# EspressoSystems/Push-CDN

Measured on AMD Instinct MI355X. Metric: broadcast_msgs_per_sec, higher is better.
Workload: dtype uint8; 1 GPU; model=gpu-broker-mesh, payload_bytes=1024, subscribers_total=10000, subscribers_per_broker=10000, topics=8, mode=broadcast, population=all, drops=0, parallelism=single-broker, global_batch=256, seq_len=1024

## Files before the change

### csrc/gpu_bindings.cpp

```cpp

#include <torch/extension.h>
#include <ATen/hip/HIPContext.h>
#include <hip/hip_runtime.h>

#include <cstdint>

#include "hip/bls_kernels.h"
#include "hip/dataplane.h"

#define CHECK_DEV(x) TORCH_CHECK(x.is_cuda(), #x " must be on the GPU")
#define CHECK_CONTIG(x) TORCH_CHECK(x.is_contiguous(), #x " must be contiguous")

static inline PairRec* pair_ptr(torch::Tensor& pairs) {
    TORCH_CHECK(pairs.dim() == 2 && pairs.size(1) == 4 && pairs.dtype() == torch::kInt32
                && pairs.is_contiguous(), "pairs must be a contiguous int32 [cap, 4] tensor");
    return (PairRec*)pairs.data_ptr<int32_t>();
}

static inline hipStream_t cur_stream() {
    return at::hip::getCurrentHIPStream().stream();
}

static inline torch::TensorOptions opts(torch::ScalarType dtype, const torch::Tensor& like) {
    return torch::TensorOptions().dtype(dtype).device(like.device());
// ... 374 lines not shown
    TORCH_CHECK(n_users >= 0 && n_peers >= 0 && ring_wpos.numel() >= n_users + n_peers,
                "ring_wpos must cover n_users + n_peers rings");
    int32_t capacity = (int32_t)pairs.size(0);
    launch_k5b_emit_direct_peers(
        disc.data_ptr<int32_t>(), owner.data_ptr<int32_t>(), origin.data_ptr<int32_t>(),
        payload_off.data_ptr<int64_t>(), payload_len.data_ptr<int32_t>(), M,
        (int32_t)n_users, (int32_t)n_peers, ring_bytes, capacity,
        (uint64_t*)ring_wpos.data_ptr<int64_t>(), n_pairs.data_ptr<int32_t>(),
        pair_ptr(pairs), (uint32_t*)drops.data_ptr<int32_t>(), cur_stream());
}

void direct_apply(torch::Tensor table_keys, torch::Tensor table_vals, torch::Tensor up_keys,
                  torch::Tensor up_owners, torch::Tensor del_keys, torch::Tensor n_failed) {
    CHECK_DEV(table_keys); CHECK_DEV(table_vals); CHECK_DEV(up_keys); CHECK_DEV(up_owners);
    CHECK_DEV(del_keys); CHECK_DEV(n_failed);
    CHECK_CONTIG(table_keys); CHECK_CONTIG(table_vals); CHECK_CONTIG(up_keys);
    CHECK_CONTIG(up_owners); CHECK_CONTIG(del_keys);
    int64_t S = table_keys.size(0);
    TORCH_CHECK(S > 0 && (S & (S - 1)) == 0, "table size must be a power of two");
    TORCH_CHECK(table_vals.numel() == S && table_keys.dtype() == torch::kInt64
                && table_vals.dtype() == torch::kInt32);
    TORCH_CHECK(up_keys.dtype() == torch::kInt64 && del_keys.dtype() == torch::kInt64
                && up_owners.dtype() == torch::kInt32 && n_failed.dtype() == torch::kInt32);
    TORCH_CHECK(up_owners.numel() == up_keys.numel() && n_failed.numel() >= 1);
    launch_k6_direct_apply((uint64_t*)table_keys.data_ptr<int64_t>(),
                           table_vals.data_ptr<int32_t>(), S,
                           (const uint64_t*)up_keys.data_ptr<int64_t>(),
                           up_owners.data_ptr<int32_t>(), (int32_t)up_keys.numel(),
                           (const uint64_t*)del_keys.data_ptr<int64_t>(),
                           (int32_t)del_keys.numel(),
                           (uint32_t*)n_failed.data_ptr<int32_t>(), cur_stream());
}

PYBIND11_MODULE(TORCH_EXTENSION_NAME, m) {
    m.def("topic_mask_origin_t", &topic_mask_origin_t,
          "K2a transposed with per-message origin: remote-origin rows keep user bits only");
    m.def("emit_direct_peers", &emit_direct_peers,
          "K5b with peer recipient slots (owner -(p+2) -> ring n_users+p, local origin only)");
    m.def("direct_apply", &direct_apply,
          "K6: batched DirectMap upserts/deletes on the device table");
    m.def("parse_batch", &parse_batch, "K4: on-device capnp parse of a message batch",
          py::arg("buf"), py::arg("offsets"), py::arg("hash_seed") = 0);
    m.def("topic_mask", &topic_mask, "K2a: per-message subscriber mask");
    m.def("assign_emit", &assign_emit, "K2b: per-user FIFO ring assignment + pair list");
    m.def("fanout", &fanout, "K3: N-way payload fan-out into egress rings");
    m.def("direct_lookup", &direct_lookup, "K5: batched direct-route hash probe");
    m.def("apply_subs", &apply_subs, "K2c: apply subscribe/unsubscribe batch to bitmap");
    m.def("bls_verify_batch", &bls_verify_batch, "K1: batched BLS-over-BN254 verification");
    m.def("compact_rings", &compact_rings,
          "K7: gather used egress-ring prefixes into one staging buffer");
    m.def("precompute_g2_lines", &precompute_g2_lines,
          "fixed-g2 Miller line coefficients for K1 v2 (once per process)");
    m.def("bls_verify_batch2", &bls_verify_batch2,
          "K1 v2: 2-lane Fp2-decomposed batched BLS verification");
    m.def("_k1_dbg_wave",
          [](torch::Tensor vks, torch::Tensor sigs, torch::Tensor msgs, torch::Tensor moff,
             torch::Tensor g2_lines, torch::Tensor rand_r, int64_t mode) {
              int32_t N = (int32_t)moff.size(0) - 1;
              auto ok = torch::zeros({N}, opts(torch::kInt32, vks));
              launch_k1_dbg_wave(vks.data_ptr<uint8_t>(), sigs.data_ptr<uint8_t>(),
                                 msgs.data_ptr<uint8_t>(), moff.data_ptr<int64_t>(),
                                 g2_lines.data_ptr<uint8_t>(),
                                 (const uint64_t*)rand_r.data_ptr<int64_t>(), N,
                                 (int32_t)mode, ok.data_ptr<int32_t>(), cur_stream());
              return ok;
          });
    m.def("bls_verify_batch_wave", &bls_verify_batch_wave,
// ... 18 lines not shown
```

### csrc/hip/dataplane.h

```cpp
#pragma once

#include <hip/hip_runtime_api.h>
#include <stdint.h>

struct alignas(16) PairRec { int32_t user; int32_t msg; int64_t dst; };
static_assert(sizeof(PairRec) == 16, "PairRec must be one dword4");

struct ParseOut {
    int32_t* disc;
    int64_t* payload_off;
    int32_t* payload_len;
    int64_t* topics_off;
    int32_t* topics_cnt;
    uint64_t* recip_hash;
    uint64_t* timestamp;
};

extern "C" {

void launch_k4_parse(const uint8_t* buf, const int64_t* offsets, int32_t M, uint64_t hash_seed,
                     ParseOut out, hipStream_t s);

void launch_k2a_topic_mask(const uint64_t* sub_bitmap, const uint8_t* buf,
                           const int64_t* topics_off, const int32_t* topics_cnt,
                           const int32_t* disc, uint64_t* mask, int32_t M, int32_t W,
                           hipStream_t s);
void launch_k2a_topic_mask_t(const uint64_t* sub_bitmap, const uint8_t* buf,
                             const int64_t* topics_off, const int32_t* topics_cnt,
                             const int32_t* disc, uint64_t* mask_t, int32_t M, int32_t W,
                             hipStream_t s);
void launch_k2a_topic_mask_origin_t(const uint64_t* sub_bitmap, const uint8_t* buf,
                                    const int64_t* topics_off, const int32_t* topics_cnt,
                                    const int32_t* disc, const int32_t* origin,
                                    uint64_t* mask_t, int32_t M, int32_t W, int32_t n_users,
                                    hipStream_t s);
void launch_k2c_apply_subs(uint64_t* sub_bitmap, const uint8_t* buf, const int64_t* topics_off,
                           const int32_t* topics_cnt, const int32_t* disc,
                           const int32_t* user_idx, int32_t M, int32_t W, hipStream_t s);

void launch_k2b_count(const uint64_t* mask, int32_t M, int32_t W, int32_t n_users,
                      int32_t* counts, hipStream_t s);
void launch_k2b_emit(const uint64_t* mask, const int64_t* payload_off,
                     const int32_t* payload_len, const int32_t* pair_base, int32_t M, int32_t W,
                     int32_t n_users, int64_t ring_bytes, uint64_t* ring_wpos, PairRec* pairs,
                     uint32_t* drops, hipStream_t s);
void launch_k2b_fused_t(const uint64_t* mask_t, const int32_t* payload_len, int32_t M,
                        int32_t W, int32_t n_users, int64_t ring_bytes, int32_t capacity,
                        int32_t uniform_rec, uint64_t* ring_wpos, int32_t* n_pairs,
// ... 16 lines not shown
                          const uint32_t* msg_seq, const int32_t* n_pairs_ptr,
                          int32_t capacity, int32_t ref_threshold, int64_t ref_base,
                          uint8_t* egress, int nt, int grid, hipStream_t s);
void launch_k3_fanout_flat2(const uint8_t* buf, const int64_t* payload_off,
                            const int32_t* payload_len, const PairRec* pairs,
                            uint32_t seq_base, const int32_t* n_pairs_ptr, int32_t capacity,
                            int32_t units_per_pair, int32_t uniform_len, uint8_t* egress,
                            int nt, int grid, hipStream_t s);
void launch_k3_fanout_flat3(const uint8_t* buf, const int64_t* payload_off,
                            const int32_t* payload_len, const PairRec* pairs,
                            const uint32_t* seq_state, const int32_t* n_pairs_ptr,
                            int32_t capacity, int32_t units_per_pair, int32_t uniform_len,
                            uint8_t* egress, int nt, int grid, hipStream_t s);
void launch_k_seq_advance(uint32_t* seq_state, int32_t m, hipStream_t s);

void launch_k5_direct_lookup(const uint64_t* table_keys, const int32_t* table_vals,
                             int64_t table_size, const uint64_t* query, int32_t N,
                             int32_t* owner, hipStream_t s);
void launch_k5b_emit_direct(const int32_t* disc, const int32_t* owner,
                            const int64_t* payload_off, const int32_t* payload_len, int32_t M,
                            int64_t ring_bytes, int32_t capacity, uint64_t* ring_wpos,
                            int32_t* n_pairs, PairRec* pairs, uint32_t* drops, hipStream_t s);
void launch_k5b_emit_direct_peers(const int32_t* disc, const int32_t* owner,
                                  const int32_t* origin, const int64_t* payload_off,
                                  const int32_t* payload_len, int32_t M, int32_t n_users,
                                  int32_t n_peers, int64_t ring_bytes, int32_t capacity,
                                  uint64_t* ring_wpos, int32_t* n_pairs, PairRec* pairs,
                                  uint32_t* drops, hipStream_t s);
void launch_k6_direct_apply(uint64_t* table_keys, int32_t* table_vals, int64_t table_size,
                            const uint64_t* up_keys, const int32_t* up_owners, int32_t n_up,
                            const uint64_t* del_keys, int32_t n_del, uint32_t* n_failed,
                            hipStream_t s);

void launch_k7_compact_rings(const uint8_t* egress, int64_t ring_bytes, const int64_t* wpos,
                             const int64_t* dst_off, uint8_t* staging, int32_t n_rings,
                             int32_t max_chunks, hipStream_t s);

}
```

### csrc/hip/dataplane.hip

```cpp

#include <hip/hip_runtime.h>
#include <stdint.h>

#include "../common/divmagic.h"
#include "dataplane.h"

#define WAVE 64
#ifndef CDN_CHECK
#define CDN_CHECK 1
#endif

#define RING_ALIGN 16ull
__host__ __device__ inline uint64_t ring_rec(int32_t len) {
    return ((uint64_t)len + 16 + (RING_ALIGN - 1)) & ~(RING_ALIGN - 1);
}

typedef unsigned int cdn_v4u __attribute__((ext_vector_type(4)));
template <int NT>
__device__ __forceinline__ void store16(void* dst, cdn_v4u v) {
    if (NT) __builtin_nontemporal_store(v, (cdn_v4u*)dst);
    else *(cdn_v4u*)dst = v;
}

__device__ __forceinline__ void store_pair(PairRec* p, int32_t u, int32_t m, int64_t d) {
// ... 502 lines not shown
            store16<NT>(egress + dsto, cdn_v4u{(uint32_t)len | REF_FLAG, seq, (uint32_t)ro,
                                               (uint32_t)(ro >> 32)});
        }
        unsigned long long inl = __ballot(live && !by_ref);
        while (inl) {
            const int j = __ffsll((long long)inl) - 1;
            inl &= inl - 1;
            const int32_t jlen = __shfl(len, j);
            const uint32_t jseq = (uint32_t)__shfl((int)seq, j);
            const int64_t joff = ((int64_t)__shfl((int)(off >> 32), j) << 32)
                                 | (uint32_t)__shfl((int)off, j);
            const int64_t jdst = ((int64_t)__shfl((int)(dsto >> 32), j) << 32)
                                 | (uint32_t)__shfl((int)dsto, j);
            copy_record<NT>(egress + jdst, buf + joff, jlen, jseq, lane, WAVE);
        }
    }
}

extern "C" {

void launch_k3_fanout_ref(const uint8_t* buf, const int64_t* payload_off,
                          const int32_t* payload_len, const PairRec* pairs,
                          const uint32_t* msg_seq, const int32_t* n_pairs_ptr,
                          int32_t capacity, int32_t ref_threshold, int64_t ref_base,
                          uint8_t* egress, int nt, int grid, hipStream_t s) {
    if (grid <= 0) grid = 4096;
    DISPATCH_NT(nt, hipLaunchKernelGGL((k3_fanout_ref_t<NT>), dim3(grid), dim3(256), 0, s, buf,
                                       payload_off, payload_len, pairs, msg_seq, n_pairs_ptr,
                                       capacity, ref_threshold, ref_base, egress));
}

}

template <int NT, bool SEQ_FROM_PTR>
__global__ void __launch_bounds__(256) k3_fanout_flat_t(
    const uint8_t* __restrict__ buf,
    const int64_t* __restrict__ payload_off,
    const int32_t* __restrict__ payload_len,
    const PairRec* __restrict__ pairs,
    uint32_t seq_base_val,
    const uint32_t* __restrict__ seq_state,
    const int32_t* __restrict__ n_pairs_ptr,
    int32_t capacity,
    int32_t units_per_pair,
    uint32_t div_magic,
    int32_t div_shift,
    int32_t uniform_len,
    uint8_t* __restrict__ egress)
{
    const uint32_t seq_base = SEQ_FROM_PTR ? seq_state[0] : seq_base_val;
    int np = *n_pairs_ptr;
    if (np > capacity) np = capacity;
    const int64_t n_units = (int64_t)np * units_per_pair;
    const int64_t stride = (int64_t)gridDim.x * blockDim.x;
    for (int64_t f = (int64_t)blockIdx.x * blockDim.x + threadIdx.x; f < n_units; f += stride) {
        const uint32_t f32 = (uint32_t)f;
        const int p = (int)(((uint64_t)f32 * div_magic) >> div_shift);
        const int unit = (int)(f32 - (uint32_t)p * (uint32_t)units_per_pair);
        const PairRec pr = pairs[p];
        if (pr.user < 0) continue;
        const int mi = pr.msg;
        const int32_t len = uniform_len > 0 ? uniform_len : payload_len[mi];
        uint8_t* dst = egress + pr.dst + (size_t)unit * 16;
        if (unit == 0) {
            store16<NT>(dst, cdn_v4u{(uint32_t)len, seq_base + (uint32_t)mi, 0u, 0u});
            continue;
        }
        const uint8_t* src = buf + payload_off[mi] + (size_t)(unit - 1) * 16;
        const int32_t coff = (unit - 1) * 16;
        if (coff + 16 <= len && (((uintptr_t)src) & 15) == 0) {
            store16<NT>(dst, *(const cdn_v4u*)src);
        } else if (coff >= len) {
            store16<NT>(dst, cdn_v4u{0u, 0u, 0u, 0u});
        } else {
            uint8_t tmp[16];
            #pragma unroll
            for (int b = 0; b < 16; ++b) tmp[b] = (coff + b < len) ? src[b] : 0;
            cdn_v4u v; memcpy(&v, tmp, 16);
            store16<NT>(dst, v);
        }
    }
}


template <bool SEQ_FROM_PTR>
static void launch_flat(const uint8_t* buf, const int64_t* payload_off,
                        const int32_t* payload_len, const PairRec* pairs, uint32_t seq_base,
                        const uint32_t* seq_state, const int32_t* n_pairs_ptr, int32_t capacity,
                        int32_t units_per_pair, int32_t uniform_len, uint8_t* egress, int nt,
                        int grid, hipStream_t s) {
    if (grid <= 0) grid = 16384;
    uint32_t dm; int32_t dsh;
    u32_div_magic(units_per_pair, &dm, &dsh);
    DISPATCH_NT(nt, hipLaunchKernelGGL((k3_fanout_flat_t<NT, SEQ_FROM_PTR>), dim3(grid),
                                       dim3(256), 0, s, buf, payload_off, payload_len, pairs,
                                       seq_base, seq_state, n_pairs_ptr, capacity,
                                       units_per_pair, dm, dsh, uniform_len, egress));
}

extern "C" __global__ void k_seq_advance(uint32_t* seq_state, int32_t m) {
    if (blockIdx.x == 0 && threadIdx.x == 0) seq_state[0] += (uint32_t)m;
}

extern "C" {

void launch_k3_fanout_flat2(const uint8_t* buf, const int64_t* payload_off,
                            const int32_t* payload_len, const PairRec* pairs,
                            uint32_t seq_base, const int32_t* n_pairs_ptr, int32_t capacity,
                            int32_t units_per_pair, int32_t uniform_len, uint8_t* egress,
                            int nt, int grid, hipStream_t s) {
    launch_flat<false>(buf, payload_off, payload_len, pairs, seq_base, nullptr, n_pairs_ptr,
                       capacity, units_per_pair, uniform_len, egress, nt, grid, s);
}
// ... 92 lines not shown

    uint64_t wpos = ring_wpos[u];
    uint32_t dropped = 0;
    for (int m = 0; m < M; ++m) {
        if (!(col[m] & bit)) continue;
        int32_t len = payload_len[m];
        uint64_t rec = ring_rec(len);
        bool fits_ring = (wpos + rec <= (uint64_t)ring_bytes);
        bool fits_cap = (slot < capacity);
        if (!fits_ring || !fits_cap) {
            if (fits_cap) { store_pair(pairs + slot, -1, m, 0); slot++; }
            dropped++;
            continue;
        }
        store_pair(pairs + slot, u, m, (int64_t)u * ring_bytes + wpos);
        slot++;
        wpos += rec;
    }
    ring_wpos[u] = wpos;
    if (dropped) atomicAdd(drops, dropped);
}

extern "C" {

void launch_k2a_topic_mask_t(const uint64_t* sub_bitmap, const uint8_t* buf,
                             const int64_t* topics_off, const int32_t* topics_cnt,
                             const int32_t* disc, uint64_t* mask_t, int32_t M, int32_t W,
                             hipStream_t s) {
    if (M <= 0) return;
    hipLaunchKernelGGL(k2a_topic_mask_t, k2a_grid(M, W), dim3(K2A_THREADS), 0, s, sub_bitmap,
                       buf, topics_off, topics_cnt, disc, mask_t, M, W);
}

#define K2B_BLK 32

extern "C" __global__ void k2b_p1_count(
    const uint64_t* __restrict__ mask_t,
    int32_t M, int32_t W, int32_t NB,
    int32_t* __restrict__ bcount)
{
    const int wave = (blockIdx.x * blockDim.x + threadIdx.x) >> 6;
    if (wave >= W * NB) return;
    const int w = wave / NB, b = wave - (int64_t)(wave / NB) * NB;
    const int lane = threadIdx.x & 63;
    const uint64_t bit = 1ull << lane;
    const uint64_t* col = mask_t + (int64_t)w * M;
    const int m0 = b * K2B_BLK, m1 = min(M, m0 + K2B_BLK);
    int c = 0;
    for (int m = m0; m < m1; ++m) c += (col[m] & bit) ? 1 : 0;
    bcount[(int64_t)b * (W * 64) + (w * 64 + lane)] = c;
}

extern "C" __global__ void k2b_p2_bases(
    const int32_t* __restrict__ bcount,
    int32_t W, int32_t NB, int32_t n_users,
    int64_t ring_bytes, int32_t capacity, int32_t uniform_rec,
    uint64_t* __restrict__ ring_wpos,
    int32_t* __restrict__ n_pairs,
    int32_t* __restrict__ pprefix,
    int32_t* __restrict__ ubase,
    int32_t* __restrict__ ufit,
    int64_t* __restrict__ udst,
    uint32_t* __restrict__ drops)
{
    const int u = blockIdx.x * blockDim.x + threadIdx.x;
    const bool active = u < n_users;
    const int lane = threadIdx.x & 63;
    int total = 0;
    if (active) {
        for (int b = 0; b < NB; ++b) {
            pprefix[(int64_t)b * (W * 64) + u] = total;
            total += bcount[(int64_t)b * (W * 64) + u];
        }
    }
    const int my_base = wave_claim_span(total, n_pairs);
    uint32_t dropped = 0;
    if (active) {
        ubase[u] = my_base;
        const uint64_t wpos = ring_wpos[u];
        const int32_t fit = (int32_t)((ring_bytes - wpos) / (uint64_t)uniform_rec);
        ufit[u] = fit;
        udst[u] = (int64_t)u * ring_bytes + (int64_t)wpos;
        int cap_room = capacity - my_base; if (cap_room < 0) cap_room = 0;
        int emitted = total; if (emitted > fit) emitted = fit; if (emitted > cap_room) emitted = cap_room;
        ring_wpos[u] = wpos + (uint64_t)emitted * uniform_rec;
        dropped = (uint32_t)(total - emitted);
    }
    for (int d = 1; d < 64; d <<= 1) dropped += __shfl_down(dropped, d);
    if (lane == 0 && dropped) atomicAdd(drops, dropped);
}

extern "C" __global__ void k2b_p3_emit(
    const uint64_t* __restrict__ mask_t,
    const int32_t* __restrict__ pprefix,
    const int32_t* __restrict__ ubase,
    const int32_t* __restrict__ ufit,
    const int64_t* __restrict__ udst,
    int32_t M, int32_t W, int32_t NB, int32_t n_users,
    int32_t capacity, int32_t uniform_rec,
    PairRec* __restrict__ pairs)
{
    const int wave = (blockIdx.x * blockDim.x + threadIdx.x) >> 6;
    if (wave >= W * NB) return;
    const int w = wave / NB, b = wave - (int64_t)(wave / NB) * NB;
    const int lane = threadIdx.x & 63;
    const int u = w * 64 + lane;
    if (u >= n_users) return;
    const uint64_t bit = 1ull << lane;
    const uint64_t* col = mask_t + (int64_t)w * M;
    int p = pprefix[(int64_t)b * (W * 64) + u];
    const int base = ubase[u], fit = ufit[u];
    const int64_t dstb = udst[u];
    const int m0 = b * K2B_BLK, m1 = min(M, m0 + K2B_BLK);
    for (int m = m0; m < m1; ++m) {
        if (!(col[m] & bit)) continue;
        const int slot = base + p;
        if (slot < capacity) {
            if (p < fit)
                store_pair(pairs + slot, u, m, dstb + (int64_t)p * uniform_rec);
            else
                store_pair(pairs + slot, -1, m, 0);
        }
// ... 228 lines not shown
                                    uint64_t* mask_t, int32_t M, int32_t W, int32_t n_users,
                                    hipStream_t s) {
    if (M <= 0) return;
    hipLaunchKernelGGL(k2a_topic_mask_origin_t, k2a_grid(M, W), dim3(K2A_THREADS), 0, s,
                       sub_bitmap, buf, topics_off, topics_cnt, disc, origin, mask_t, M, W,
                       n_users);
}

void launch_k5b_emit_direct_peers(
    const int32_t* disc, const int32_t* owner, const int32_t* origin,
    const int64_t* payload_off, const int32_t* payload_len, int32_t M, int32_t n_users,
    int32_t n_peers, int64_t ring_bytes, int32_t capacity, uint64_t* ring_wpos,
    int32_t* n_pairs, PairRec* pairs, uint32_t* drops, hipStream_t s) {
    if (M <= 0) return;
    int threads = 256, blocks = (M + threads - 1) / threads;
    hipLaunchKernelGGL(k5b_emit_direct_peers, dim3(blocks), dim3(threads), 0, s, disc, owner,
                       origin, payload_off, payload_len, M, n_users, n_peers, ring_bytes,
                       capacity, ring_wpos, n_pairs, pairs, drops);
}

void launch_k6_direct_apply(uint64_t* table_keys, int32_t* table_vals, int64_t table_size,
                            const uint64_t* up_keys, const int32_t* up_owners, int32_t n_up,
                            const uint64_t* del_keys, int32_t n_del, uint32_t* n_failed,
                            hipStream_t s) {
    const int total = n_up + n_del;
    if (total <= 0) return;
    int threads = 256, blocks = (total + threads - 1) / threads;
    hipLaunchKernelGGL(k6_direct_apply, dim3(blocks), dim3(threads), 0, s, table_keys,
                       table_vals, table_size, up_keys, up_owners, n_up, del_keys, n_del,
                       n_failed);
}

}
```

### pushcdn_amd/broker/gpu_engine.py

```python

from __future__ import annotations

import os

from dataclasses import dataclass
from typing import Dict, List, Optional, Tuple

import torch

from ..utils.keyhash import fnv1a64
from ..utils.log import get_logger

log = get_logger("gpu-engine")

RING_ALIGN = 16
REF_FLAG = 0x80000000


def ring_rec(length: int) -> int:
    return (length + 16 + (RING_ALIGN - 1)) & ~(RING_ALIGN - 1)


@dataclass
class TickStats:
    n_messages: int = 0
    n_broadcast: int = 0
    n_direct: int = 0
    n_deliveries: int = 0
    n_drops: int = 0


class GpuBrokerEngine:
    def __init__(
        self,
        device: str = "cuda:0",
        n_users: int = 10_000,
        ring_bytes: int = 1 << 21,
        direct_table_size: int = 1 << 16,
        use_gpu_ops: Optional[bool] = None,
        fanout_wire: bool = False,
        pair_capacity: int = 4 << 20,
        nt_fanout: bool = True,
        direct_enabled: bool = True,
        hash_seed: int = 0,
        n_peer_slots: int = 0,
        ref_threshold: Optional[int] = None,
    ) -> None:
        assert n_peer_slots >= 0
        self.n_peer_slots = n_peer_slots
        self.n_recipients = n_users + n_peer_slots
        self.pair_capacity = pair_capacity
        self._flat_max_rec = int(os.environ.get("PUSHCDN_FLAT_MAX_REC", "4096"))
        flat_units = self._flat_max_rec // 16 + 1
        assert 1 <= flat_units <= (1 << 21), "PUSHCDN_FLAT_MAX_REC too large"
        assert pair_capacity * flat_units < (1 << 31), (
            f"pair_capacity {pair_capacity} x {flat_units} flat units/record "
            "must stay below 2^31")
        self.nt_fanout = nt_fanout
        self.direct_enabled = direct_enabled
        self.hash_seed = hash_seed & ((1 << 64) - 1)
        self.fanout_wire = fanout_wire
        self.device = torch.device(device)
        self.is_cuda = self.device.type == "cuda"
        if use_gpu_ops is None:
            use_gpu_ops = self.is_cuda
        self.use_gpu_ops = use_gpu_ops
        if self.use_gpu_ops:
            from ..ops import get_gpu_ops

            self._ops = get_gpu_ops()
        else:
            self._ops = None

        assert ring_bytes % 16 == 0
        self.n_users = n_users
        self.ring_bytes = ring_bytes
        R = self.n_recipients
        self.W = (R + 63) // 64

        dev = self.device
        self.sub_bitmap = torch.zeros((256, self.W), dtype=torch.int64, device=dev)
        self.egress = torch.zeros(R * ring_bytes, dtype=torch.uint8, device=dev)
        self.ring_wpos = torch.zeros(R, dtype=torch.int64, device=dev)
        self.direct_keys = torch.zeros(direct_table_size, dtype=torch.int64, device=dev)
        self.direct_vals = torch.zeros(direct_table_size, dtype=torch.int32, device=dev)
        self._direct_entries: Dict[int, int] = {}
        self._direct_pubkeys: Dict[int, bytes] = {}
        self._direct_tombstones: set = set()
        self._direct_failed = torch.zeros(1, dtype=torch.int32, device=dev)
        if ref_threshold is not None:
            assert fanout_wire, "ref_threshold requires fanout_wire=True"
            assert 1 <= ref_threshold < REF_FLAG
            assert ring_rec(ref_threshold - 1) <= ring_bytes, (
                f"ref_threshold {ref_threshold}: an inline message just below it "
                f"does not fit a {ring_bytes}-byte ring")
        self.ref_threshold = ref_threshold
        self._ref_batches: List[bytes] = []
        self._ref_base = 0
        self.seq = 0
        self.total = TickStats()
        self._staging_dev: Optional[torch.Tensor] = None
        self._staging_host: Optional[torch.Tensor] = None
        if self.use_gpu_ops:
            o32 = dict(dtype=torch.int32, device=dev)
            self._pairs = torch.empty((pair_capacity, 4), **o32)
            self._drops = torch.zeros(1, **o32)
            self._n_pairs = torch.zeros(1, **o32)
            self._seq_dev = torch.zeros(1, **o32)
            self._graphs: Dict[Tuple[int, int, int], object] = {}


    def subscribe(self, user_idx: int, topics: List[int]) -> None:
        w, bit = user_idx >> 6, 1 << (user_idx & 63)
        bit = bit - (1 << 64) if bit >= (1 << 63) else bit
        for t in topics:
            self.sub_bitmap[t & 0xFF, w] |= bit

    def unsubscribe(self, user_idx: int, topics: List[int]) -> None:
        w, bit = user_idx >> 6, 1 << (user_idx & 63)
        bit = bit - (1 << 64) if bit >= (1 << 63) else bit
        for t in topics:
            self.sub_bitmap[t & 0xFF, w] &= ~bit

    def subscribe_all(self, topics: List[int]) -> None:
        if self.n_peer_slots:
            full = self._user_bit_words().to(self.device)
            for t in topics:
                self.sub_bitmap[t & 0xFF] |= full
            return
        full = torch.full((self.W,), -1, dtype=torch.int64)
        tail = self.n_users & 63
        if tail:
            full[-1] = (1 << tail) - 1
        for t in topics:
            self.sub_bitmap[t & 0xFF] = full.to(self.device)

    def _user_bit_words(self) -> torch.Tensor:
        words = torch.zeros(self.W, dtype=torch.int64)
        nfull = self.n_users >> 6
        words[:nfull] = -1
        tail = self.n_users & 63
# ... 201 lines not shown
        self._ref_base = 0

    def _k2b_block_scratch(self, M: int):
        NB = (M + 31) // 32
        W64 = self.W * 64
        cur = getattr(self, "_k2b_scratch", None)
        if cur is not None and cur[0] >= NB:
            return cur[1]
        o32 = dict(dtype=torch.int32, device=self.device)
        bufs = (
            torch.empty(NB * W64, **o32),
            torch.empty(NB * W64, **o32),
            torch.empty(W64, **o32),
            torch.empty(W64, **o32),
            torch.empty(W64, dtype=torch.int64, device=self.device),
        )
        self._k2b_scratch = (NB, bufs)
        return bufs

    def _assign_emit(self, ops, mask_t, payload_len, rec: int, M: int) -> None:
        if rec and self.use_gpu_ops:
            bcount, pprefix, ubase, ufit, udst = self._k2b_block_scratch(M)
            ops.assign_emit_blocks_t(
                mask_t, self.ring_wpos, self.ring_bytes, self.n_recipients,
                bcount, pprefix, ubase, ufit, udst,
                self._pairs, self._drops, self._n_pairs, rec,
            )
        else:
            ops.assign_emit_fused_t(
                mask_t, payload_len, self.ring_wpos, self.ring_bytes, self.n_recipients,
                self._pairs, self._drops, self._n_pairs, rec,
            )

    def _tick_gpu(self, buf: torch.Tensor, offsets: torch.Tensor,
                  uniform_wire_len: Optional[int] = None, origin=None,
                  ref_base: int = 0) -> TickStats:
        ops = self._ops
        M = offsets.shape[0] - 1
        disc, payload_off, payload_len, topics_off, topics_cnt, recip_hash, _ts = ops.parse_batch(
            buf, offsets, self.hash_seed
        )
        peer_plane = self.n_peer_slots > 0 or origin is not None
        if peer_plane:
            origin = self._origin_tensor(origin, M)
            mask_t = ops.topic_mask_origin_t(self.sub_bitmap, buf, topics_off, topics_cnt,
                                             disc, origin, self.n_users)
        else:
            mask_t = ops.topic_mask_t(self.sub_bitmap, buf, topics_off, topics_cnt, disc)
        if self.fanout_wire:
            payload_off = offsets[:-1].contiguous()
            payload_len = (offsets[1:] - offsets[:-1]).to(torch.int32).contiguous()
        self._n_pairs.zero_()
        uniform = self.fanout_wire and uniform_wire_len is not None
        thr = self.ref_threshold
        ring_len = payload_len
        if thr is not None:
            if uniform and uniform_wire_len >= thr:
                uniform = False
            if not uniform:
                ring_len = torch.where(payload_len >= thr, 0, payload_len).to(torch.int32)
        rec = ring_rec(uniform_wire_len) if uniform else 0
        self._assign_emit(ops, mask_t, ring_len, rec, M)
        if self.direct_enabled:
            owner = ops.direct_lookup(self.direct_keys, self.direct_vals, recip_hash)
            if peer_plane:
                ops.emit_direct_peers(disc, owner, origin, payload_off, ring_len,
                                      self.ring_bytes, self.n_users, self.n_peer_slots,
                                      self.ring_wpos, self._n_pairs, self._pairs,
                                      self._drops)
            else:
                ops.emit_direct(disc, owner, payload_off, ring_len, self.ring_bytes,
# ... 76 lines not shown
                torch.tensor(offsets[1:], dtype=torch.int64)
                - torch.tensor(offsets[:-1], dtype=torch.int64)
            ).to(torch.int32)
        thr = self.ref_threshold
        ring_len = pr.payload_len if thr is None else ref.ring_lengths(pr.payload_len, thr)

        def fan(p_user, p_msg, p_dst):
            if thr is None:
                ref.fanout(batch, pr.payload_off, pr.payload_len, p_user, p_msg, p_dst,
                           seq, arr)
            else:
                ref.fanout_ref(batch, pr.payload_off, pr.payload_len, p_user, p_msg, p_dst,
                               seq, arr, thr, ref_base)

        pair_user, pair_msg, pair_dst, drops = ref.assign_emit(
            mask, ring_len, self.ring_wpos, self.ring_bytes, self.n_recipients
        )
        seq = torch.arange(self.seq, self.seq + M, dtype=torch.int32)
        self.seq += M
        arr = bytearray(self.egress.numpy().tobytes())
        fan(pair_user, pair_msg, pair_dst)
        owner = ref.direct_lookup(self.direct_keys, self.direct_vals, pr.recip_hash)
        d_user, d_msg, d_dst, d_drops = ref.emit_direct_peers(
            pr.disc, owner, origin, ring_len, self.ring_wpos, self.ring_bytes,
            self.n_users, self.n_peer_slots)
        fan(d_user, d_msg, d_dst)
        self.egress.copy_(torch.frombuffer(arr, dtype=torch.uint8))
        return TickStats(n_messages=M, n_deliveries=int(pair_user.shape[0]),
                         n_drops=drops + d_drops)


    def drain_cursors(self) -> torch.Tensor:
        self._discard_ref_batches()
        wpos = self.ring_wpos.detach().clone().to("cpu")
        self.ring_wpos.zero_()
        return wpos

    def drain_compact(self) -> Tuple[torch.Tensor, torch.Tensor, torch.Tensor]:
        self._discard_ref_batches()
        return self._drain_compact()

    def drain_compact_ref(self):
        batches = self._ref_batches
        self._discard_ref_batches()
        if len(batches) == 1:
            refbuf = batches[0]
        else:
            refbuf = b"".join(bytes(b) for b in batches)
        return (*self._drain_compact(), refbuf)

    def _drain_compact(self) -> Tuple[torch.Tensor, torch.Tensor, torch.Tensor]:
        if not self.use_gpu_ops:
            wpos = self.ring_wpos.detach().clone()
            self.ring_wpos.zero_()
            offsets = torch.zeros(self.n_recipients + 1, dtype=torch.int64)
            torch.cumsum(wpos, 0, out=offsets[1:])
            total = int(offsets[-1])
            staging = torch.empty(total, dtype=torch.uint8)
            for u in range(self.n_recipients):
                n = int(wpos[u])
                if n:
                    s = u * self.ring_bytes
                    staging[int(offsets[u]):int(offsets[u + 1])] = self.egress[s:s + n]
            return wpos, offsets, staging
        wpos_dev = self.ring_wpos
        wpos = wpos_dev.detach().to("cpu")
# ... 65 lines not shown
```

Before: 393,600 msgs/s.

## Add fused uniform broadcast tick with dense tile fan-out and fused cursor drain

Adds a single host entry point that runs parse, topic mask, per-tile k2b assignment and fan-out back to back from preallocated scratch, so the per-tick Python dispatch and tensor allocation go away. Fully subscribed 32-message tiles are written as a dense image broadcast to every user's ring, and only leftover tiles are emitted as sparse pairs. Cursor drain becomes one kernel plus a pinned async copy. Tick stats no longer report deliveries or drops, and the path applies only to uniform, non-direct, non-peer ticks.

```diff
diff --git a/csrc/common/tick_geom.h b/csrc/common/tick_geom.h
--- /dev/null
+++ b/csrc/common/tick_geom.h
@@ -0,0 +1,29 @@
+#pragma once
+
+#include <stdint.h>
+
+#define K2B_BLK 32
+
+#define DENSE_THREADS 256
+#define DENSE_MAX_V 8
+#define DENSE_GROUP 8
+struct DenseGeom { int32_t n_chunks; int32_t chunk_units; };
+static inline DenseGeom dense_geom(int32_t units_per_rec) {
+    const int32_t cap = DENSE_THREADS * DENSE_MAX_V;
+    const int32_t image = units_per_rec * K2B_BLK;
+    DenseGeom g;
+    g.n_chunks = (image + cap - 1) / cap;
+    g.chunk_units = ((image + g.n_chunks - 1) / g.n_chunks + 63) & ~63;
+    return g;
+}
+static inline int64_t dense_grid_x(int32_t n_users, int32_t group, int32_t n_chunks) {
+    return ((int64_t)n_users + group - 1) / group * n_chunks;
+}
+
+static inline int64_t k2b_blocks(int64_t M) { return (M + K2B_BLK - 1) / K2B_BLK; }
+static inline int64_t uniform_tick_scratch64(int64_t M, int64_t W, int64_t units_per_rec) {
+    return 4 * M + W * M + k2b_blocks(M) * W * 64 + W * 64 + 2 * M * units_per_rec;
+}
+static inline int64_t uniform_tick_scratch32(int64_t M, int64_t W) {
+    return 3 * M + 3 * k2b_blocks(M) * W * 64 + 2 * W * 64;
+}
diff --git a/csrc/gpu_bindings.cpp b/csrc/gpu_bindings.cpp
--- a/csrc/gpu_bindings.cpp
+++ b/csrc/gpu_bindings.cpp
@@ -430,7 +430,97 @@
                            (uint32_t*)n_failed.data_ptr<int32_t>(), cur_stream());
 }
 
+void tick_uniform_broadcast(torch::Tensor buf, torch::Tensor offsets, uint64_t hash_seed,
+                            torch::Tensor sub_bitmap, torch::Tensor ring_wpos,
+                            int64_t ring_bytes, int64_t n_users, torch::Tensor pairs,
+                            torch::Tensor drops, torch::Tensor n_pairs, torch::Tensor n_sparse,
+                            torch::Tensor scratch64, torch::Tensor scratch32,
+                            int64_t uniform_len, int64_t seq_base, torch::Tensor egress,
+                            int64_t nt, int64_t dense) {
+    CHECK_DEV(buf); CHECK_CONTIG(buf); CHECK_DEV(offsets); CHECK_CONTIG(offsets);
+    CHECK_DEV(sub_bitmap); CHECK_CONTIG(sub_bitmap); CHECK_DEV(ring_wpos); CHECK_CONTIG(ring_wpos);
+    CHECK_DEV(egress); CHECK_CONTIG(egress); CHECK_DEV(scratch64); CHECK_DEV(scratch32);
+    CHECK_DEV(drops); CHECK_DEV(n_pairs); CHECK_DEV(n_sparse);
+    TORCH_CHECK(buf.dtype() == torch::kUInt8 && offsets.dtype() == torch::kInt64
+                && egress.dtype() == torch::kUInt8);
+    TORCH_CHECK(sub_bitmap.dim() == 2 && sub_bitmap.size(0) == 256);
+    const int64_t M = offsets.size(0) - 1, W = sub_bitmap.size(1);
+    if (M <= 0) return;
+    TORCH_CHECK(uniform_len >= 0 && uniform_len < (int64_t(1) << 30));
+    const int64_t rec = (uniform_len + 16 + 15) & ~int64_t(15);
+    TORCH_CHECK(ring_bytes % 16 == 0 && n_users >= 0 && n_users <= W * 64
+                && ring_wpos.numel() >= n_users && ring_wpos.dtype() == torch::kInt64
+                && egress.numel() >= n_users * ring_bytes,
+                "rings do not cover n_users");
+    TORCH_CHECK(buf.numel() >= M * uniform_len, "batch shorter than M uniform messages");
+    check_flat_shape(pairs, rec / 16);
+    TORCH_CHECK(M * (rec / 16) < (int64_t(1) << 31)
+                && dense_grid_x((int32_t)n_users, DENSE_GROUP, dense_geom((int32_t)(rec / 16)).n_chunks)
+                       * k2b_blocks(M) < (int64_t(1) << 31),
+                "batch too large for the dense fan-out");
+    TORCH_CHECK(scratch64.dtype() == torch::kInt64 && scratch32.dtype() == torch::kInt32
+                && scratch64.is_contiguous() && scratch32.is_contiguous()
+                && (uintptr_t)scratch64.data_ptr<int64_t>() % 16 == 0
+                && scratch64.numel() >= uniform_tick_scratch64(M, W, rec / 16)
+                && scratch32.numel() >= uniform_tick_scratch32(M, W),
+                "fused tick scratch too small");
+    UniformTick t;
+    t.buf = buf.data_ptr<uint8_t>();
+    t.offsets = offsets.data_ptr<int64_t>();
+    t.M = (int32_t)M;
+    t.hash_seed = hash_seed;
+    t.sub_bitmap = (const uint64_t*)sub_bitmap.data_ptr<int64_t>();
+    t.W = (int32_t)W;
+    t.n_users = (int32_t)n_users;
+    t.ring_bytes = ring_bytes;
+    t.capacity = (int32_t)pairs.size(0);
+    t.uniform_len = (int32_t)uniform_len;
+    t.rec = (int32_t)rec;
+    t.seq_base = (uint32_t)seq_base;
+    t.ring_wpos = (uint64_t*)ring_wpos.data_ptr<int64_t>();
+    t.n_pairs = n_pairs.data_ptr<int32_t>();
+    t.n_sparse = n_sparse.data_ptr<int32_t>();
+    t.pairs = pair_ptr(pairs);
+    t.drops = (uint32_t*)drops.data_ptr<int32_t>();
+    t.scratch64 = scratch64.data_ptr<int64_t>();
+    t.scratch32 = scratch32.data_ptr<int32_t>();
+    t.egress = egress.data_ptr<uint8_t>();
+    t.nt = (int)nt;
+    t.dense = (int)dense;
+    launch_tick_uniform_broadcast(&t, cur_stream());
+}
+
+std::vector<int64_t> uniform_tick_scratch_sizes(int64_t M, int64_t W, int64_t rec) {
+    return {uniform_tick_scratch64(M, W, rec / 16), uniform_tick_scratch32(M, W)};
+}
+
+void drain_cursors(torch::Tensor ring_wpos, torch::Tensor staging, torch::Tensor host) {
+    CHECK_DEV(ring_wpos); CHECK_CONTIG(ring_wpos); CHECK_DEV(staging); CHECK_CONTIG(staging);
+    TORCH_CHECK(!host.is_cuda() && host.is_pinned() && host.is_contiguous(),
+                "host must be a pinned CPU tensor");
+    TORCH_CHECK(ring_wpos.dtype() == torch::kInt64 && staging.dtype() == torch::kInt64
+                && host.dtype() == torch::kInt64);
+    const int64_t n = ring_wpos.numel();
+    TORCH_CHECK(staging.numel() >= n && host.numel() >= n && n <= INT32_MAX);
+    if (n == 0) return;
+    hipStream_t s = cur_stream();
+    launch_drain_cursors(ring_wpos.data_ptr<int64_t>(), staging.data_ptr<int64_t>(), (int32_t)n,
+                         s);
+    hipError_t e = hipMemcpyAsync(host.data_ptr<int64_t>(), staging.data_ptr<int64_t>(),
+                                  (size_t)n * 8, hipMemcpyDeviceToHost, s);
+    TORCH_CHECK(e == hipSuccess, "drain_cursors copy: ", hipGetErrorString(e));
+    e = hipStreamSynchronize(s);
+    TORCH_CHECK(e == hipSuccess, "drain_cursors sync: ", hipGetErrorString(e));
+}
+
 PYBIND11_MODULE(TORCH_EXTENSION_NAME, m) {
+    m.def("tick_uniform_broadcast", &tick_uniform_broadcast,
+          "fused uniform broadcast tick: K4, K2a, K2b tiles, dense + sparse fan-out");
+    m.def("uniform_tick_scratch_sizes", &uniform_tick_scratch_sizes,
+          "(int64, int32) scratch elements tick_uniform_broadcast needs for (M, W, rec)");
+    m.def("drain_cursors", &drain_cursors,
+          "fused drain: cursors -> pinned host buffer, cursors zeroed, stream synchronised",
+          py::call_guard<py::gil_scoped_release>());
     m.def("topic_mask_origin_t", &topic_mask_origin_t,
           "K2a transposed with per-message origin: remote-origin rows keep user bits only");
     m.def("emit_direct_peers", &emit_direct_peers,
diff --git a/csrc/hip/dataplane.h b/csrc/hip/dataplane.h
--- a/csrc/hip/dataplane.h
+++ b/csrc/hip/dataplane.h
@@ -2,6 +2,8 @@
 
 #include <hip/hip_runtime_api.h>
 #include <stdint.h>
+
+#include "../common/tick_geom.h"
 
 struct alignas(16) PairRec { int32_t user; int32_t msg; int64_t dst; };
 static_assert(sizeof(PairRec) == 16, "PairRec must be one dword4");
@@ -14,6 +16,31 @@
     int32_t* topics_cnt;
     uint64_t* recip_hash;
     uint64_t* timestamp;
+};
+
+struct UniformTick {
+    const uint8_t* buf;
+    const int64_t* offsets;
+    int32_t M;
+    uint64_t hash_seed;
+    const uint64_t* sub_bitmap;
+    int32_t W;
+    int32_t n_users;
+    int64_t ring_bytes;
+    int32_t capacity;
+    int32_t uniform_len;
+    int32_t rec;
+    uint32_t seq_base;
+    uint64_t* ring_wpos;
+    int32_t* n_pairs;
+    int32_t* n_sparse;
+    PairRec* pairs;
+    uint32_t* drops;
+    int64_t* scratch64;
+    int32_t* scratch32;
+    uint8_t* egress;
+    int nt;
+    int dense;
 };
 
 extern "C" {
@@ -96,6 +123,10 @@
                             const uint64_t* del_keys, int32_t n_del, uint32_t* n_failed,
                             hipStream_t s);
 
+void launch_tick_uniform_broadcast(const UniformTick* t, hipStream_t s);
+
+void launch_drain_cursors(int64_t* ring_wpos, int64_t* staging, int32_t n, hipStream_t s);
+
 void launch_k7_compact_rings(const uint8_t* egress, int64_t ring_bytes, const int64_t* wpos,
                              const int64_t* dst_off, uint8_t* staging, int32_t n_rings,
                              int32_t max_chunks, hipStream_t s);
diff --git a/csrc/hip/dataplane.hip b/csrc/hip/dataplane.hip
--- a/csrc/hip/dataplane.hip
+++ b/csrc/hip/dataplane.hip
@@ -558,6 +558,19 @@
 
 }
 
+__device__ __forceinline__ cdn_v4u payload_unit(const uint8_t* __restrict__ msg, int32_t coff,
+                                                int32_t len)
+{
+    const uint8_t* src = msg + coff;
+    if (coff + 16 <= len && (((uintptr_t)src) & 15) == 0) return *(const cdn_v4u*)src;
+    if (coff >= len) return cdn_v4u{0u, 0u, 0u, 0u};
+    uint8_t tmp[16];
+    #pragma unroll
+    for (int b = 0; b < 16; ++b) tmp[b] = (coff + b < len) ? src[b] : 0;
+    cdn_v4u v; memcpy(&v, tmp, 16);
+    return v;
+}
+
 template <int NT, bool SEQ_FROM_PTR>
 __global__ void __launch_bounds__(256) k3_fanout_flat_t(
     const uint8_t* __restrict__ buf,
@@ -592,19 +605,7 @@
             store16<NT>(dst, cdn_v4u{(uint32_t)len, seq_base + (uint32_t)mi, 0u, 0u});
             continue;
         }
-        const uint8_t* src = buf + payload_off[mi] + (size_t)(unit - 1) * 16;
-        const int32_t coff = (unit - 1) * 16;
-        if (coff + 16 <= len && (((uintptr_t)src) & 15) == 0) {
-            store16<NT>(dst, *(const cdn_v4u*)src);
-        } else if (coff >= len) {
-            store16<NT>(dst, cdn_v4u{0u, 0u, 0u, 0u});
-        } else {
-            uint8_t tmp[16];
-            #pragma unroll
-            for (int b = 0; b < 16; ++b) tmp[b] = (coff + b < len) ? src[b] : 0;
-            cdn_v4u v; memcpy(&v, tmp, 16);
-            store16<NT>(dst, v);
-        }
+        store16<NT>(dst, payload_unit(buf + payload_off[mi], (unit - 1) * 16, len));
     }
 }
 
@@ -763,9 +764,8 @@
                        buf, topics_off, topics_cnt, disc, mask_t, M, W);
 }
 
-#define K2B_BLK 32
-
-extern "C" __global__ void k2b_p1_count(
+
+__device__ __forceinline__ void k2b_p1_body(
     const uint64_t* __restrict__ mask_t,
     int32_t M, int32_t W, int32_t NB,
     int32_t* __restrict__ bcount)
@@ -780,6 +780,48 @@
     int c = 0;
     for (int m = m0; m < m1; ++m) c += (col[m] & bit) ? 1 : 0;
     bcount[(int64_t)b * (W * 64) + (w * 64 + lane)] = c;
+}
+
+extern "C" __global__ void k2b_p1_count(
+    const uint64_t* __restrict__ mask_t, int32_t M, int32_t W, int32_t NB,
+    int32_t* __restrict__ bcount)
+{
+    k2b_p1_body(mask_t, M, W, NB, bcount);
+}
+
+struct K2bUser { int32_t base; int32_t fit; int64_t dst; };
+
+__device__ __forceinline__ K2bUser k2b_p2_body(
+    const int32_t* __restrict__ bcount,
+    int u, bool active, int32_t W, int32_t NB,
+    int64_t ring_bytes, int32_t capacity, int32_t uniform_rec,
+    uint64_t* __restrict__ ring_wpos,
+    int32_t* __restrict__ n_pairs,
+    int32_t* __restrict__ pprefix,
+    uint32_t* __restrict__ drops)
+{
+    const int lane = threadIdx.x & 63;
+    int total = 0;
+    if (active) {
+        for (int b = 0; b < NB; ++b) {
+            pprefix[(int64_t)b * (W * 64) + u] = total;
+            total += bcount[(int64_t)b * (W * 64) + u];
+        }
+    }
+    K2bUser r{wave_claim_span(total, n_pairs), 0, 0};
+    uint32_t dropped = 0;
+    if (active) {
+        const uint64_t wpos = ring_wpos[u];
+        r.fit = (int32_t)((ring_bytes - wpos) / (uint64_t)uniform_rec);
+        r.dst = (int64_t)u * ring_bytes + (int64_t)wpos;
+        int cap_room = capacity - r.base; if (cap_room < 0) cap_room = 0;
+        int emitted = total; if (emitted > r.fit) emitted = r.fit; if (emitted > cap_room) emitted = cap_room;
+        ring_wpos[u] = wpos + (uint64_t)emitted * uniform_rec;
+        dropped = (uint32_t)(total - emitted);
+    }
+    for (int d = 1; d < 64; d <<= 1) dropped += __shfl_down(dropped, d);
+    if (lane == 0 && dropped) atomicAdd(drops, dropped);
+    return r;
 }
 
 extern "C" __global__ void k2b_p2_bases(
@@ -796,29 +838,13 @@
 {
     const int u = blockIdx.x * blockDim.x + threadIdx.x;
     const bool active = u < n_users;
-    const int lane = threadIdx.x & 63;
-    int total = 0;
+    const K2bUser r = k2b_p2_body(bcount, u, active, W, NB, ring_bytes, capacity, uniform_rec,
+                                  ring_wpos, n_pairs, pprefix, drops);
     if (active) {
-        for (int b = 0; b < NB; ++b) {
-            pprefix[(int64_t)b * (W * 64) + u] = total;
-            total += bcount[(int64_t)b * (W * 64) + u];
-        }
-    }
-    const int my_base = wave_claim_span(total, n_pairs);
-    uint32_t dropped = 0;
-    if (active) {
-        ubase[u] = my_base;
-        const uint64_t wpos = ring_wpos[u];
-        const int32_t fit = (int32_t)((ring_bytes - wpos) / (uint64_t)uniform_rec);
-        ufit[u] = fit;
-        udst[u] = (int64_t)u * ring_bytes + (int64_t)wpos;
-        int cap_room = capacity - my_base; if (cap_room < 0) cap_room = 0;
-        int emitted = total; if (emitted > fit) emitted = fit; if (emitted > cap_room) emitted = cap_room;
-        ring_wpos[u] = wpos + (uint64_t)emitted * uniform_rec;
-        dropped = (uint32_t)(total - emitted);
-    }
-    for (int d = 1; d < 64; d <<= 1) dropped += __shfl_down(dropped, d);
-    if (lane == 0 && dropped) atomicAdd(drops, dropped);
+        ubase[u] = r.base;
+        ufit[u] = r.fit;
+        udst[u] = r.dst;
+    }
 }
 
 extern "C" __global__ void k2b_p3_emit(
@@ -1113,3 +1139,228 @@
 }
 
 }
+
+extern "C" __global__ void k2b_p1_count_z(
+    const uint64_t* __restrict__ mask_t, int32_t M, int32_t W, int32_t NB,
+    int32_t* __restrict__ bcount, int32_t* __restrict__ n_pairs, int32_t* __restrict__ n_sparse)
+{
+    if (blockIdx.x == 0 && threadIdx.x == 0) { *n_pairs = 0; *n_sparse = 0; }
+    k2b_p1_body(mask_t, M, W, NB, bcount);
+}
+
+extern "C" __global__ void k2b_p2_tiles(
+    const int32_t* __restrict__ bcount,
+    int32_t M, int32_t W, int32_t NB, int32_t n_users,
+    int64_t ring_bytes, int32_t capacity, int32_t uniform_rec, int32_t use_dense,
+    uint64_t* __restrict__ ring_wpos,
+    int32_t* __restrict__ n_pairs,
+    int32_t* __restrict__ n_sparse,
+    int32_t* __restrict__ pprefix,
+    int32_t* __restrict__ tslot,
+    int64_t* __restrict__ tdst,
+    int32_t* __restrict__ ulim,
+    int32_t* __restrict__ usbase,
+    int64_t* __restrict__ udst,
+    uint32_t* __restrict__ drops)
+{
+    const int u = blockIdx.x * blockDim.x + threadIdx.x;
+    const bool active = u < n_users;
+    const K2bUser r = k2b_p2_body(bcount, u, active, W, NB, ring_bytes, capacity, uniform_rec,
+                                  ring_wpos, n_pairs, pprefix, drops);
+    int cap_room = capacity - r.base; if (cap_room < 0) cap_room = 0;
+    const int lim = r.fit < cap_room ? r.fit : cap_room;
+    int n_sp = 0;
+    if (active) {
+        int p = 0;
+        for (int b = 0; b < NB; ++b) {
+            const int64_t i = (int64_t)b * (W * 64) + u;
+            const int cnt = bcount[i];
+            const int nm = min(M - b * K2B_BLK, K2B_BLK);
+            const bool dense = use_dense && cnt == nm && p + cnt <= lim;
+            tdst[i] = dense ? r.dst + (int64_t)p * uniform_rec : -1;
+            tslot[i] = n_sp;
+            if (!dense) n_sp += max(0, min(cnt, lim - p));
+            p += cnt;
+        }
+    }
+    const int sbase = wave_claim_span(n_sp, n_sparse);
+    if (active) {
+        ulim[u] = lim;
+        usbase[u] = sbase;
+        udst[u] = r.dst;
+    }
+}
+
+extern "C" __global__ void k2b_p3_sparse(
+    const uint64_t* __restrict__ mask_t,
+    const int32_t* __restrict__ bcount,
+    const int32_t* __restrict__ pprefix,
+    const int32_t* __restrict__ tslot,
+    const int64_t* __restrict__ tdst,
+    const int32_t* __restrict__ ulim,
+    const int32_t* __restrict__ usbase,
+    const int64_t* __restrict__ udst,
+    int32_t M, int32_t W, int32_t NB, int32_t n_users, int32_t uniform_rec,
+    PairRec* __restrict__ pairs)
+{
+    const int wave = (blockIdx.x * blockDim.x + threadIdx.x) >> 6;
+    if (wave >= W * NB) return;
+    const int w = wave / NB, b = wave - (wave / NB) * NB;
+    const int lane = threadIdx.x & 63;
+    const int u = w * 64 + lane;
+    int p0 = 0, lim = 0, slot0 = 0;
+    int64_t dstb = 0;
+    bool sparse = false;
+    if (u < n_users) {
+        const int64_t i = (int64_t)b * (W * 64) + u;
+        p0 = pprefix[i];
+        lim = ulim[u];
+        sparse = tdst[i] < 0 && bcount[i] > 0 && p0 < lim;
+        slot0 = usbase[u] + tslot[i];
+        dstb = udst[u];
+    }
+    unsigned long long todo = __ballot(sparse);
+    if (!todo) return;
+    const int m0 = b * K2B_BLK, nm = min(M - m0, K2B_BLK);
+    const uint64_t word = lane < nm ? mask_t[(int64_t)w * M + m0 + lane] : 0ull;
+    while (todo) {
+        const int j = __ffsll((long long)todo) - 1;
+        todo &= todo - 1;
+        const int jp0 = __shfl(p0, j), jlim = __shfl(lim, j), jslot = __shfl(slot0, j);
+        const int64_t jdst = ((int64_t)__shfl((int)(dstb >> 32), j) << 32)
+                             | (uint32_t)__shfl((int)dstb, j);
+        const bool bit = (word >> j) & 1ull;
+        const unsigned long long mb = __ballot(bit);
+        const int rank = __popcll(mb & ((1ull << lane) - 1ull));
+        const int p = jp0 + rank;
+        if (bit && p < jlim)
+            store_pair(pairs + jslot + rank, w * 64 + j, m0 + lane,
+                       jdst + (int64_t)p * uniform_rec);
+    }
+}
+
+extern "C" __global__ void k3d_image(
+    const uint8_t* __restrict__ buf,
+    const int64_t* __restrict__ offsets,
+    int32_t M, int32_t units_per_rec, uint32_t div_magic, int32_t div_shift,
+    int32_t uniform_len, uint32_t seq_base,
+    cdn_v4u* __restrict__ image)
+{
+    const uint32_t i = blockIdx.x * blockDim.x + threadIdx.x;
+    if (i >= (uint32_t)(M * units_per_rec)) return;
+    const int m = (int)(((uint64_t)i * div_magic) >> div_shift);
+    const int q = (int)i - m * units_per_rec;
+    image[i] = q == 0 ? cdn_v4u{(uint32_t)uniform_len, seq_base + (uint32_t)m, 0u, 0u}
+                      : payload_unit(buf + offsets[m], (q - 1) * 16, uniform_len);
+}
+
+__global__ void __launch_bounds__(DENSE_THREADS) k3_fanout_dense(
+    const cdn_v4u* __restrict__ image,
+    const int64_t* __restrict__ tdst,
+    int32_t M, int32_t NB, int32_t users64, int32_t n_users, int32_t units_per_rec,
+    int32_t n_chunks, int32_t chunk_units, int32_t group,
+    uint8_t* __restrict__ egress)
+{
+    const int per_group = NB * n_chunks;
+    const int g = blockIdx.x / per_group, bc = blockIdx.x - g * per_group;
+    const int b = bc / n_chunks, c = bc - b * n_chunks;
+    const int m0 = b * K2B_BLK, nm = min(M - m0, K2B_BLK);
+    const int lo = c * chunk_units + (int)threadIdx.x;
+    const int hi = min(nm * units_per_rec, (c + 1) * chunk_units);
+    if (lo >= hi) return;
+    const cdn_v4u* __restrict__ img = image + (size_t)m0 * units_per_rec;
+    cdn_v4u v[DENSE_MAX_V];
+    #pragma unroll
+    for (int k = 0; k < DENSE_MAX_V; ++k) {
+        const int unit = lo + k * DENSE_THREADS;
+        v[k] = unit < hi ? img[unit] : cdn_v4u{0u, 0u, 0u, 0u};
+    }
+    const int64_t* __restrict__ trow = tdst + (int64_t)b * users64;
+    const int u1 = min(n_users, (g + 1) * group);
+    for (int u = g * group; u < u1; ++u) {
+        const int64_t d = trow[u];
+        if (d < 0) continue;
+        uint8_t* dst = egress + d + (size_t)lo * 16;
+        #pragma unroll
+        for (int k = 0; k < DENSE_MAX_V; ++k)
+            if (lo + k * DENSE_THREADS < hi)
+                store16<0>(dst + (size_t)k * (DENSE_THREADS * 16), v[k]);
+    }
+}
+
+extern "C" __global__ void k_drain_cursors(int64_t* __restrict__ ring_wpos,
+                                           int64_t* __restrict__ staging, int32_t n)
+{
+    const int i = blockIdx.x * blockDim.x + threadIdx.x;
+    if (i >= n) return;
+    staging[i] = ring_wpos[i];
+    ring_wpos[i] = 0;
+}
+
+extern "C" {
+
+void launch_tick_uniform_broadcast(const UniformTick* t, hipStream_t s) {
+    const int32_t M = t->M, W = t->W;
+    if (M <= 0) return;
+    const int32_t NB = (int32_t)k2b_blocks(M);
+    const int64_t U = (int64_t)W * 64, T = (int64_t)NB * U;
+    const int32_t units = t->rec / 16;
+    int64_t* p64 = t->scratch64;
+    cdn_v4u* image = (cdn_v4u*)p64;  p64 += 2 * (int64_t)M * units;
+    int64_t* payload_off = p64;  p64 += M;
+    int64_t* topics_off = p64;   p64 += M;
+    int64_t* recip_hash = p64;   p64 += M;
+    int64_t* timestamp = p64;    p64 += M;
+    uint64_t* mask_t = (uint64_t*)p64;  p64 += (int64_t)W * M;
+    int64_t* tdst = p64;         p64 += T;
+    int64_t* udst = p64;
+    int32_t* p32 = t->scratch32;
+    int32_t* disc = p32;         p32 += M;
+    int32_t* payload_len = p32;  p32 += M;
+    int32_t* topics_cnt = p32;   p32 += M;
+    int32_t* bcount = p32;       p32 += T;
+    int32_t* pprefix = p32;      p32 += T;
+    int32_t* tslot = p32;        p32 += T;
+    int32_t* ulim = p32;         p32 += U;
+    int32_t* usbase = p32;
+
+    launch_k4_parse(t->buf, t->offsets, M, t->hash_seed,
+                    ParseOut{disc, payload_off, payload_len, topics_off, topics_cnt,
+                             (uint64_t*)recip_hash, (uint64_t*)timestamp}, s);
+    launch_k2a_topic_mask_t(t->sub_bitmap, t->buf, topics_off, topics_cnt, disc, mask_t, M, W, s);
+
+    const int threads = 256;
+    const int blocks_wb = (W * NB * 64 + threads - 1) / threads;
+    const int blocks_u = (t->n_users + threads - 1) / threads;
+    hipLaunchKernelGGL(k2b_p1_count_z, dim3(blocks_wb), dim3(threads), 0, s, mask_t, M, W, NB,
+                       bcount, t->n_pairs, t->n_sparse);
+    hipLaunchKernelGGL(k2b_p2_tiles, dim3(blocks_u), dim3(threads), 0, s, bcount, M, W, NB,
+                       t->n_users, t->ring_bytes, t->capacity, t->rec, t->dense ? 1 : 0,
+                       t->ring_wpos, t->n_pairs, t->n_sparse, pprefix, tslot, tdst, ulim, usbase,
+                       udst, t->drops);
+    hipLaunchKernelGGL(k2b_p3_sparse, dim3(blocks_wb), dim3(threads), 0, s, mask_t, bcount,
+                       pprefix, tslot, tdst, ulim, usbase, udst, M, W, NB, t->n_users, t->rec,
+                       t->pairs);
+    if (t->dense) {
+        const DenseGeom geo = dense_geom(units);
+        uint32_t dm; int32_t dsh;
+        u32_div_magic(units, &dm, &dsh);
+        hipLaunchKernelGGL(k3d_image, dim3((M * units + threads - 1) / threads), dim3(threads),
+                           0, s, t->buf, t->offsets, M, units, dm, dsh, t->uniform_len,
+                           t->seq_base, image);
+        const dim3 grid((uint32_t)(dense_grid_x(t->n_users, DENSE_GROUP, geo.n_chunks) * NB));
+        hipLaunchKernelGGL(k3_fanout_dense, grid, dim3(DENSE_THREADS), 0, s, image, tdst, M, NB,
+                           (int32_t)U, t->n_users, units, geo.n_chunks, geo.chunk_units,
+                           DENSE_GROUP, t->egress);
+    }
+    launch_flat<false>(t->buf, t->offsets, payload_len, t->pairs, t->seq_base, nullptr,
+                       t->n_sparse, t->capacity, units, t->uniform_len, t->egress, t->nt, 0, s);
+}
+
+void launch_drain_cursors(int64_t* ring_wpos, int64_t* staging, int32_t n, hipStream_t s) {
+    if (n <= 0) return;
+    hipLaunchKernelGGL(k_drain_cursors, dim3((n + 255) / 256), dim3(256), 0, s, ring_wpos,
+                       staging, n);
+}
+
+}
diff --git a/pushcdn_amd/broker/gpu_engine.py b/pushcdn_amd/broker/gpu_engine.py
--- a/pushcdn_amd/broker/gpu_engine.py
+++ b/pushcdn_amd/broker/gpu_engine.py
@@ -45,6 +45,7 @@
         hash_seed: int = 0,
         n_peer_slots: int = 0,
         ref_threshold: Optional[int] = None,
+        fused_tick: bool = True,
     ) -> None:
         assert n_peer_slots >= 0
         self.n_peer_slots = n_peer_slots
@@ -58,6 +59,8 @@
             "must stay below 2^31")
         self.nt_fanout = nt_fanout
         self.direct_enabled = direct_enabled
+        self.fused_tick = fused_tick
+        self.fused_ticks = 0
         self.hash_seed = hash_seed & ((1 << 64) - 1)
         self.fanout_wire = fanout_wire
         self.device = torch.device(device)
@@ -107,6 +110,10 @@
             self._drops = torch.zeros(1, **o32)
             self._n_pairs = torch.zeros(1, **o32)
             self._seq_dev = torch.zeros(1, **o32)
+            self._n_sparse = torch.zeros(1, **o32)
+            self._dense_fanout = True
+            self._fused_scratch = None
+            self._drain_bufs = None
             self._graphs: Dict[Tuple[int, int, int], object] = {}
 
 
@@ -374,11 +381,40 @@
                 self._pairs, self._drops, self._n_pairs, rec,
             )
 
+    def _fused_tick_ok(self, uniform_wire_len: Optional[int], origin) -> bool:
+        return (self.fused_tick and self.fanout_wire and uniform_wire_len is not None
+                and not self.direct_enabled and self.n_peer_slots == 0
+                and origin is None and self.ref_threshold is None
+                and ring_rec(uniform_wire_len) <= self._flat_max_rec)
+
+    def _tick_fused(self, buf: torch.Tensor, offsets: torch.Tensor,
+                    uniform_wire_len: int, M: int) -> TickStats:
+        ops = self._ops
+        n64, n32 = ops.uniform_tick_scratch_sizes(M, self.W, ring_rec(uniform_wire_len))
+        s64, s32 = self._fused_scratch or (None, None)
+        if s64 is None or s64.numel() < n64 or s32.numel() < n32:
+            s64 = torch.empty(max(n64, 0 if s64 is None else s64.numel()),
+                              dtype=torch.int64, device=self.device)
+            s32 = torch.empty(max(n32, 0 if s32 is None else s32.numel()),
+                              dtype=torch.int32, device=self.device)
+            self._fused_scratch = (s64, s32)
+        seq_base = self.seq
+        self.seq += M
+        ops.tick_uniform_broadcast(
+            buf, offsets, self.hash_seed, self.sub_bitmap, self.ring_wpos, self.ring_bytes,
+            self.n_recipients, self._pairs, self._drops, self._n_pairs, self._n_sparse,
+            s64, s32, uniform_wire_len, seq_base, self.egress,
+            1 if self.nt_fanout else 0, 1 if self._dense_fanout else 0)
+        self.fused_ticks += 1
+        return TickStats(n_messages=M)
+
     def _tick_gpu(self, buf: torch.Tensor, offsets: torch.Tensor,
                   uniform_wire_len: Optional[int] = None, origin=None,
                   ref_base: int = 0) -> TickStats:
         ops = self._ops
         M = offsets.shape[0] - 1
+        if M > 0 and self._fused_tick_ok(uniform_wire_len, origin):
+            return self._tick_fused(buf, offsets, uniform_wire_len, M)
         disc, payload_off, payload_len, topics_off, topics_cnt, recip_hash, _ts = ops.parse_batch(
             buf, offsets, self.hash_seed
         )
@@ -521,6 +557,15 @@
 
     def drain_cursors(self) -> torch.Tensor:
         self._discard_ref_batches()
+        if self.fused_tick and self.use_gpu_ops and self.is_cuda:
+            if self._drain_bufs is None:
+                self._drain_bufs = (
+                    torch.empty_like(self.ring_wpos),
+                    torch.empty(self.ring_wpos.shape, dtype=torch.int64, pin_memory=True),
+                )
+            staging, host = self._drain_bufs
+            self._ops.drain_cursors(self.ring_wpos, staging, host)
+            return host.clone()
         wpos = self.ring_wpos.detach().clone().to("cpu")
         self.ring_wpos.zero_()
         return wpos
```

Result: faster. 439,900 msgs/s, median of 6 (+11.7%).
